# dkogan/libdogleg

Hardware: NVIDIA B200
Metric: dogleg_iterations_per_sec (higher is better)
Workload: dtype f64

## Files before the change

### libdogleg_b200/csrc/dlb_device.h

```cpp
#pragma once
#include <cuda_runtime.h>
#include <cstdint>
#include "dlb_taskplan.h"
#include "dlb_common.cuh"

struct __align__(16) DlbClsInfo { int k, m0, nm, r0; };
struct __align__(16) DlbLeaf { long long off; int c0, nc, r, rp, fcls0, ncls; };
struct __align__(16) DlbSmallTask { int k, m0, nm, r0; long long goff, Goff; };

struct DlbSparseDev
{
  int n, m, ncls, ntasks;
  const int* cls_ptr;
  const int* cls_rows;
  const int* cls_loc;
  const int* cls_front;
  const int* task_cls;
  const int* task_m0;
  const int* task_m1;
  const long long* task_goff;
  const long long* task_Goff;
  const int* mem_col;
  const unsigned int* mem_pos;
  const int* ginv_ptr;
// ... 28 lines not shown
  const int* w;
  const long long* src_ptr;
  const long long* gs_base;
  const int* gs_ld;
};

struct DlbFrontDev
{
  int n, nsuper;
  const int* sn_first;
  const int* rows_ptr;
  const int* rows;
  const int* rel;
  const int* sn_parent;
  const int* child_ptr;
  const int* child_list;
  const long long* front_off;
  const int* fcls_ptr;
  const int* fcls_list;
  const int* cls_task_ptr;
  const int* level_sn;
  const int* perm;
  const DlbLeaf* leaf;
  const unsigned int* leaf_pos; const unsigned int* leaf_kl; const unsigned int* leaf_loc;
  int leaf_ps, leaf_lw;
  int leaf_max_nc;
  long long ytot;
  const long long* heavy_tmp_off;
  double* heavy_tmp;
  DlbGather fg;
  DlbGather sg;
  const char* sg_flag;
};

struct DlbBigFront { long long off; int r, nc, col0, sn; long long inv_off; };

#define DLB_TRIAL_PART 8
#define DLB_TRIAL_PROF_MAX 62
enum { DLB_TRIAL_CAUCHY = 0, DLB_TRIAL_GN = 1, DLB_TRIAL_INTERP = 2 };
struct DlbPublished { DlbScalars sc; unsigned long long seq; };
struct DlbTrial
{
  int nlev; const int* level_ptr; const long long* level_gt; const long long* level_sg; const long long* level_tmp;
  int max_rows, max_cols, any_solve_gather;
  int small_tail;
  const double* Jtx; const double* p_from; const double* Gpart; double* cauchy; double* gn;
  double norm2_Jtx, norm2_cauchy, norm2_gn; int have_cauchy, have_gn;
  double* step; double* p_to; double* h_p_to;
  double* fronts; double* ywork; double* zperm;
  double* part; unsigned int* bar; long long* minor; long long* minor_next;
  DlbScalars* sc; DlbPublished* pub; unsigned long long seq;
  double delta, lambda;
  const int* eg_ptr; const unsigned int* eg_dst; const int* eg_sptr; const int* eg_src;
  unsigned long long* prof;
};
size_t dlb_trial_smem_bytes(int max_rows);
int  dlb_trial_threads(int max_rows);
int  dlb_trial_max_grid(int max_rows, int sm_count);
int  dlb_launch_trial(const DlbSparseDev& S, const DlbFrontDev& F, const DlbTrial& T, int grid, cudaStream_t st);

void dlb_launch_sparse_grad(const DlbSparseDev& S, const double* Jx, const double* x, double* gpart,
                            double* n2part, double* Jtx, double* part, unsigned int* counter,
                            DlbScalars* sc, int sm_count, cudaStream_t st);
int  dlb_sparse_n2part_size(const DlbSparseDev& S, int sm_count);
struct DlbPublished;
int  dlb_launch_sparse_eval_pass(const DlbSparseDev& S, const double* Jx, const double* x, double* Gpart, double* gpart,
                                 double* n2part, int sm_count, cudaStream_t st);
void dlb_launch_sparse_eval_reduce(const DlbSparseDev& S, const double* gpart, const double* n2part, int n2count, double* Jtx,
                                   double* part, unsigned int* counter, DlbScalars* sc, DlbPublished* pub, unsigned long long seq,
                                   int n2_behind_Jtx, int sm_count, cudaStream_t st);
void dlb_launch_sparse_jv(const DlbSparseDev& S, const double* Jx, const double* v, double* part,
                          unsigned int* counter, double* dst, int sm_count, cudaStream_t st);
void dlb_launch_sparse_jv_quad(const DlbSparseDev& S, const double* Jx, const double* Gpart, const double* v, double* part,
                               unsigned int* counter, double* dst, int sm_count, cudaStream_t st);
void dlb_launch_sparse_assemble(const DlbSparseDev& S, const double* Jx, double* Gpart, int all_small,
                                int sm_count, cudaStream_t st);

void dlb_launch_leaf_fronts(const DlbFrontDev& F, const DlbSparseDev& S, int q0, int q1, const double* Jx,
                            double* fronts, double lambda, long long* minor, int max_rows, int eliminate,
                            int sm_count, cudaStream_t st);
void dlb_launch_leaf_fronts_mma(const DlbFrontDev& F, const DlbSparseDev& S, int q0, int q1, const double* Jx,
                                double* fronts, double lambda, long long* minor, int max_rows, int max_pairs, int eliminate,
                                int sm_count, cudaStream_t st);
void dlb_launch_leaf_solve_fwd(const DlbFrontDev& F, int q0, int q1, const double* fronts, const double* rhs,
                               double* ywork, double* zperm, int nrhs, int sm_count, cudaStream_t st);
void dlb_launch_leaf_solve_bwd(const DlbFrontDev& F, int q0, int q1, const double* fronts, double* zperm,
                               int nrhs, int sm_count, cudaStream_t st);

void dlb_launch_front_level(const DlbFrontDev& F, const DlbSparseDev& S, int l0, int l1,
                            double* fronts, const double* Gpart, double lambda,
                            long long* minor, int max_rows, int skip_elimination, cudaStream_t st);
void dlb_bigfront_factor_batch(const DlbBigFront* d_descs, int nfronts, int max_r, int max_nc, double* fronts, double* inv,
                               int* cnt, long long* minor, cudaStream_t st, double* n_launch);
void dlb_launch_extend_gather(const DlbGather& G, long long t0, long long t1, double* pool, int accumulate, cudaStream_t st);
void dlb_launch_zero_bigfronts(const DlbBigFront* d_descs, int nfronts, int max_r, double* fronts, cudaStream_t st);
void dlb_launch_solve_fwd_level(const DlbFrontDev& F, int l0, int l1, const double* fronts,
                                const double* rhs , double* ywork,
                                double* zperm, int nrhs, int max_rows, int max_cols, cudaStream_t st);
void dlb_launch_solve_bwd_level(const DlbFrontDev& F, int l0, int l1, const double* fronts,
                                double* zperm, int nrhs, int max_rows, int max_cols, cudaStream_t st);
void dlb_launch_fronts_to_dense(const DlbFrontDev& F, const double* fronts, double* out, cudaStream_t st);

void dlb_launch_bigsolve_fwd(const DlbFrontDev& F, const DlbBigFront* d_descs, int nfronts, int max_r, int max_nc,
                             const double* fronts, const double* inv, const double* rhs, double* ywork, double* zperm, int nrhs,
                             cudaStream_t st);
long long dlb_bigsolve_partial_size(int r, int nc);
// ... 28 lines not shown
```

### libdogleg_b200/csrc/dlb_engine.cu

```cuda
#include "dlb_common.cuh"
#include "dlb_device.h"
#include "dlb_symbolic.h"
#include "dlb_gatherplan.h"
#include "dlb_taskplan.h"
#include "dogleg_gpu.h"
#include <vector>
#include <string>
#include <cstring>
#include <cstdlib>
#include <climits>
#include <algorithm>
#include <type_traits>
#include <mutex>
#include <chrono>
#include <thread>

static_assert(sizeof(DlbScalars) == sizeof(dlb_scalars_t), "scalar block mirrors must agree");
#define DLB_SMALL_FRONT_MAX 158

static thread_local std::string g_last_error;
static int g_device = 0;
extern "C" const char* dogleg_gpu_last_error(void) { return g_last_error.c_str(); }
extern "C" const char* dogleg_gpu_version(void)    { return "libdogleg-b200 0.1 (sm_100a)"; }
extern "C" void dlb_set_error(const char* msg)     { g_last_error = msg ? msg : ""; }
// ... 85 lines not shown
{
  double *h_p = 0, *h_x = 0, *h_Jtx = 0, *h_cauchy = 0, *h_gn = 0, *h_step = 0, *h_J = 0;
  int    *h_Jp = 0, *h_Ji = 0;
  double *d_p = 0, *d_x = 0, *d_Jtx = 0, *d_cauchy = 0, *d_gn = 0, *d_step = 0, *d_J = 0;
  double norm2_x = 0;
  double* d_G = 0; bool have_G = false;
  double norm2_Jtx = 0, norm2_cauchy = 0, norm2_gn = 0; bool have_cauchy = false, have_gn = false;
};

struct dlb_engine
{
  int type = 0, N = 0, M = 0, packed = 0, upper = 0, device = 0, sm_count = DLB_SM_COUNT_FALLBACK;
  unsigned int nnz = 0;
  size_t Jcount = 0;
  cudaStream_t st = 0;
  cudaStream_t st_copy = 0; cudaEvent_t ev_copy = 0, ev_idle = 0;
  Slot slot[2];
  DlbScalars* d_sc = 0;
  dlb_scalars_t* h_sc = 0;
  DlbPublished* h_pub = 0; DlbPublished* d_pub = 0; unsigned long long seq = 0;
  double* d_part = 0; unsigned int* d_counter = 0;
  long long* d_minor = 0; long long* h_minor = 0;
  DlbSymbolic* sym = 0;
  DlbSparseDev S{}; DlbFrontDev F{};
  std::vector<void*> dev_allocs;
  std::vector<int> level_ptr;
  std::vector<long long> level_gt_ptr;
  std::vector<long long> level_tmp_size;
  std::vector<long long> level_sg_ptr;
  bool any_solve_gather = false;
  std::vector<int> level_mid;
  std::vector<std::vector<DlbBigFront>> level_big;
  std::vector<int> level_big_ptr, level_big_max_r, level_big_max_nc;
  const DlbBigFront* d_big_descs = 0;
  int* d_big_cnt = 0;
  double* d_biginv = 0;
  const long long* d_big_part_off = 0; double* d_big_partial = 0;
  int max_small_rows = 0;
  int max_front_rows = 0, max_front_cols = 0;
  std::vector<int> level_small_rows, level_rows, level_cols;
  int nleaf = 0, leaf_max_rows = 0;
  bool leaf_mma = false;
  int leaf_max_pairs = 0;
  double *d_gpart = 0, *d_n2part = 0, *d_jvpart = 0, *d_fronts = 0, *d_ywork = 0, *d_zperm = 0;
  bool G_shared = false;
  bool G_global = false;
  long long Goff_total = 0;
  bool fused_eval = false, fused_trial = false;
  int trial_grid = 0;
  const int* d_level_ptr = 0; const long long *d_level_gt = 0, *d_level_sg = 0, *d_level_tmp = 0;
  double* d_trial_part = 0; unsigned int* d_bar = 0;
  unsigned int trial_parity = 0; bool minor_dirty = true;
  const int *d_eg_ptr = 0, *d_eg_sptr = 0, *d_eg_src = 0; const unsigned int* d_eg_dst = 0;
  unsigned long long* d_prof = 0;
  double *d_rhs = 0; int rhs_cap = 0;
  bool sharded = false; int M_total = 0, col_begin = 0;
  bool gather = false;
  long long slice_off = 0;
  std::vector<long long> rank_cb, rank_m, rank_off, rank_nnz;
  double* d_fronts_asm = 0;
  double n_allreduce = 0, allreduce_bytes = 0;
  bool pattern_set = false;
  bool pattern_verified = false;
  bool host_inputs = true;
  std::vector<int> pat_sample;
  unsigned long long pat_hash = 0;
  std::vector<int> pat_full_p, pat_full_i;
  std::vector<int> perm_used; int postorder_used = 0;
  double *d_work = 0, *d_xAx = 0;
  int factor_slot = -1; double factor_lambda = 0;
  int asm_slot = 0;
  bool jv_quad = true;
  bool lazy_p = false;
  double n_launch = 0, n_h2d = 0, n_d2h = 0, n_factor = 0;
  bool timing = false; double phase_ms[8] = {0};
  cudaEvent_t ev0 = 0, ev1 = 0;
};

template<class T> static int dev_upload(dlb_engine* e, const std::vector<T>& v, const T** out)
{
  T* d = 0;
  const size_t bytes = std::max<size_t>(v.size(), 1) * sizeof(T);
  CU(cudaMalloc(&d, bytes));
  e->dev_allocs.push_back(d);
  if(!v.empty()) CU(cudaMemcpyAsync(d, v.data(), v.size() * sizeof(T), cudaMemcpyHostToDevice, e->st));
  *out = d;
  return 0;
}
template<class T> static int dev_alloc(dlb_engine* e, size_t count, T** out)
{
  T* d = 0;
  CU(cudaMalloc(&d, std::max<size_t>(count, 1) * sizeof(T)));
  e->dev_allocs.push_back(d);
  *out = d;
  return 0;
}

static int upload_big_descs(dlb_engine* e)
{
  std::vector<DlbBigFront> all;
  const size_t nlev = e->level_big.size();
  e->level_big_ptr.assign(nlev + 1, 0); e->level_big_max_r.assign(nlev, 0); e->level_big_max_nc.assign(nlev, 0);
  for(size_t l = 0; l < nlev; l++)
  {
    for(const DlbBigFront& b : e->level_big[l])
    {
// ... 721 lines not shown
  e->fused_trial = false;
  {
    const char* ft = getenv("DOGLEG_GPU_FUSED_TRIAL");
    bool can = e->fused_eval && !e->gather && e->nleaf == 0 && Y.nlevels > 0 && Y.nlevels <= 256 &&
               Y.max_front_rows <= DLB_SMALL_FRONT_MAX && !(ft && atoi(ft) == 0);
    for(size_t l = 0; can && l < e->level_big.size(); l++) if(!e->level_big[l].empty()) can = false;
    if(can)
    {
      const int limit = dlb_trial_max_grid(Y.max_front_rows, e->sm_count);
      int want = e->sm_count;
      for(int l = 0; l < Y.nlevels; l++) want = std::max(want, Y.level_ptr[l+1] - Y.level_ptr[l]);
      want = std::max(want, (S.nbig + S.nasm_small + dlb_trial_threads(Y.max_front_rows) / 32 - 1) / (dlb_trial_threads(Y.max_front_rows) / 32));
      e->trial_grid = std::min(limit, std::min(want, 4 * e->sm_count));
      if(e->trial_grid >= 1)
      {
        std::vector<long long> lgt(e->level_gt_ptr), lsg(e->level_sg_ptr), ltmp(e->level_tmp_size);
        lgt.resize(2 * (size_t)Y.nlevels + 1, 0); lsg.resize(2 * (size_t)Y.nlevels + 1, 0); ltmp.resize((size_t)Y.nlevels, 0);
        int r2 = 0;
        r2 |= dev_upload(e, Y.level_ptr, &e->d_level_ptr);
        r2 |= dev_upload(e, lgt, &e->d_level_gt); r2 |= dev_upload(e, lsg, &e->d_level_sg); r2 |= dev_upload(e, ltmp, &e->d_level_tmp);
        {
          std::vector<int> eg_ptr(Y.nsuper + 1, 0), eg_sptr{0}, eg_src;
          std::vector<unsigned int> eg_dst;
          struct Ent { unsigned int dst; int src; };
          std::vector<Ent> ents;
          bool fits = Goff < (1ll << 31);
          for(int sn = 0; sn < Y.nsuper && fits; sn++)
          {
            ents.clear();
            for(int ci = Y.fcls_ptr[sn]; ci < Y.fcls_ptr[sn+1]; ci++)
            {
              const int c = Y.fcls_list[ci];
              const int k = Y.cls_ptr[c+1] - Y.cls_ptr[c];
              const int* loc = Y.cls_loc.data() + Y.cls_ptr[c];
              for(int a = 0, q = 0; a < k; a++)
                for(int b = 0; b <= a; b++, q++)
                {
                  const int la = loc[a], lb = loc[b];
                  const unsigned int row = (unsigned int)std::max(la, lb), col = (unsigned int)std::min(la, lb);
                  for(int t = cls_task_ptr[c]; t < cls_task_ptr[c+1]; t++) ents.push_back({row | (col << 16), (int)(task_Goff[t] + q)});
                }
            }
            std::stable_sort(ents.begin(), ents.end(), [](const Ent& x, const Ent& y) { return x.dst < y.dst; });
            for(size_t i = 0; i < ents.size(); i++)
            {
              if(i == 0 || ents[i].dst != ents[i-1].dst) { if(i) eg_sptr.push_back((int)eg_src.size()); eg_dst.push_back(ents[i].dst); }
              eg_src.push_back(ents[i].src);
            }
            if(!ents.empty()) eg_sptr.push_back((int)eg_src.size());
            eg_ptr[sn+1] = (int)eg_dst.size();
            if(eg_src.size() > (size_t)1 << 30) fits = false;
          }
          if(!fits) { g_last_error = "element lists too large"; r2 = 1; }
          r2 |= dev_upload(e, eg_ptr, &e->d_eg_ptr); r2 |= dev_upload(e, eg_dst, &e->d_eg_dst);
          r2 |= dev_upload(e, eg_sptr, &e->d_eg_sptr); r2 |= dev_upload(e, eg_src, &e->d_eg_src);
        }
        r2 |= dev_alloc(e, (size_t)e->trial_grid * DLB_TRIAL_PART, &e->d_trial_part);
        r2 |= dev_alloc(e, (size_t)4, &e->d_bar);
        { const char* pe = getenv("DOGLEG_GPU_TRIAL_PROF"); e->d_prof = 0; if(pe && atoi(pe) != 0) r2 |= dev_alloc(e, (size_t)DLB_TRIAL_PROF_MAX + 1, &e->d_prof); }
        if(r2) { g_last_error = "out of device memory for the trial kernel's workspace"; return -1; }
        CU(cudaMemsetAsync(e->d_bar, 0, 4 * sizeof(unsigned int), e->st));
        e->fused_trial = true;
      }
    }
  }
  CU(cudaStreamSynchronize(e->st));
  e->pattern_set = true;
  e->pattern_verified = true;
  if(verbose)
  {
    const auto t_end = std::chrono::steady_clock::now();
    size_t fr = 0, tot = 0; cudaMemGetInfo(&fr, &tot);
    fprintf(stderr, "libdogleg-b200: pattern N=%d M=%d: %d classes, %d supernodes, %d levels, nnz(L)=%lld, fronts %.2f GB, "
            "max front %d; symbolic %.2f s, index build + upload %.2f s; device memory in use %.1f GB; fused evaluation %d, trial kernel %d (grid %d)\n",
            e->N, Mtot, Y.ncls, Y.nsuper, Y.nlevels, (long long)Y.nnzL(), 8e-9 * (double)Y.front_off[Y.nsuper], Y.max_front_rows,
            std::chrono::duration<double>(t_sym - t_begin).count(), std::chrono::duration<double>(t_end - t_sym).count(),
            1e-9 * (double)(tot - fr), (int)e->fused_eval, (int)e->fused_trial, e->trial_grid);
  }
  return 0;
}

extern "C" int dlb_engine_upload_p(dlb_engine_t* e, int s)
{
  cudaSetDevice(e->device);
  Slot& L = e->slot[s & 1];
  CU(cudaMemcpyAsync(L.d_p, L.h_p, sizeof(double) * e->N, cudaMemcpyHostToDevice, e->st));
  e->n_h2d += sizeof(double) * e->N;
  return 0;
}

static thread_local struct { dlb_engine* e; int slot; size_t wJ, wx; } g_fill = {0, 0, 0, 0};
#define DLB_FILL_MIN_BYTES (1u << 20)
extern "C" void dlb_engine_begin_host_fill(dlb_engine_t* e, int s)
{
  g_fill.e = 0;
  if(!e->host_inputs || e->type == DOGLEG_DENSE_PRODUCTS) return;
  cudaSetDevice(e->device);
  if(cudaEventRecord(e->ev_idle, e->st) != cudaSuccess || cudaStreamWaitEvent(e->st_copy, e->ev_idle, 0) != cudaSuccess) { cudaGetLastError(); return; }
  g_fill.e = e; g_fill.slot = s & 1; g_fill.wJ = 0; g_fill.wx = 0;
}
static void fill_copy_upto(dlb_engine* e, Slot& L, size_t nJ, size_t nx, bool all)
{
  nJ = std::min(nJ, e->Jcount); nx = std::min(nx, (size_t)e->M);
  if(nx > g_fill.wx && (all || (nx - g_fill.wx) * sizeof(double) >= DLB_FILL_MIN_BYTES))
  {
    cudaMemcpyAsync(L.d_x + (e->gather ? e->col_begin : 0) + g_fill.wx, L.h_x + g_fill.wx, sizeof(double) * (nx - g_fill.wx),
                    cudaMemcpyHostToDevice, e->st_copy);
    g_fill.wx = nx;
// ... 605 lines not shown
{
  cudaSetDevice(e->device);
  Slot& A = e->slot[from & 1]; Slot& B = e->slot[to & 1];
  if(ensure_G(e, from)) return -1;
  {
    PhaseTimer tm(e, 6);
    dlb_launch_step(step_type, delta, A.d_p, A.d_Jtx, A.d_cauchy, A.d_gn, e->N, B.d_step, B.d_p,
                    e->d_part, e->d_counter, e->d_sc, e->sm_count, e->st);
    e->n_launch += step_type == DLB_STEP_INTERPOLATED ? 2 : 1;
    if(launch_norm2_Jv(e, A, B.d_step, &e->d_sc->norm2_Jstep)) return -1;
  }
  if(!e->lazy_p)
  {
    PhaseTimer tm(e, 7);
    CU(cudaMemcpyAsync(B.h_p, B.d_p, sizeof(double) * e->N, cudaMemcpyDeviceToHost, e->st));
    e->n_d2h += sizeof(double) * e->N;
  }
  return sync_scalars(e);
}

extern "C" int dlb_engine_has_trial(const dlb_engine_t* e) { return e->fused_trial ? 1 : 0; }
extern "C" int dlb_engine_has_fused_eval(const dlb_engine_t* e) { return e->fused_eval ? 1 : 0; }
extern "C" int dlb_engine_trial(dlb_engine_t* e, int from, int to, double delta, double lambda)
{
  cudaSetDevice(e->device);
  if(!e->fused_trial) { g_last_error = "dlb_engine_trial: this engine has no fused trial kernel (dlb_engine_has_trial)"; return -1; }
  Slot& A = e->slot[from & 1]; Slot& B = e->slot[to & 1];
  if(!A.have_G) { g_last_error = "dlb_engine_trial: the starting point has not been evaluated"; return -1; }
  if(A.have_gn && (e->factor_slot != (from & 1))) A.have_gn = false;
  if(!A.have_gn) e->factor_slot = -1;
  if(e->minor_dirty)
  {
    static const long long big2[2] = {LLONG_MAX, LLONG_MAX};
    CU(cudaMemcpyAsync(e->d_minor, big2, sizeof(big2), cudaMemcpyHostToDevice, e->st));
    e->minor_dirty = false;
  }
  DlbTrial T;
  memset(&T, 0, sizeof(T));
  T.nlev = (int)e->level_ptr.size() - 1; T.level_ptr = e->d_level_ptr; T.level_gt = e->d_level_gt;
  T.level_sg = e->d_level_sg; T.level_tmp = e->d_level_tmp;
  T.max_rows = e->max_front_rows; T.max_cols = e->max_front_cols; T.any_solve_gather = e->any_solve_gather ? 1 : 0;
  T.small_tail = 2 * (size_t)e->N * sizeof(double) <= dlb_trial_smem_bytes(e->max_front_rows) ? 1 : 0;
  T.Jtx = A.d_Jtx; T.p_from = A.d_p; T.Gpart = A.d_G; T.cauchy = A.d_cauchy; T.gn = A.d_gn;
  T.norm2_Jtx = A.norm2_Jtx; T.norm2_cauchy = A.norm2_cauchy; T.norm2_gn = A.norm2_gn;
  T.have_cauchy = A.have_cauchy ? 1 : 0; T.have_gn = A.have_gn ? 1 : 0;
  T.step = B.d_step; T.p_to = B.d_p; T.h_p_to = e->lazy_p ? NULL : B.h_p;
  T.fronts = e->d_fronts; T.ywork = e->d_ywork; T.zperm = e->d_zperm;
  T.part = e->d_trial_part; T.bar = e->d_bar;
  T.minor = e->d_minor + (e->trial_parity & 1); T.minor_next = e->d_minor + ((e->trial_parity + 1) & 1);
  e->trial_parity++;
  T.sc = e->d_sc; T.pub = e->d_pub; T.seq = ++e->seq;
  T.delta = delta; T.lambda = lambda; T.prof = e->d_prof;
  T.eg_ptr = e->d_eg_ptr; T.eg_dst = e->d_eg_dst; T.eg_sptr = e->d_eg_sptr; T.eg_src = e->d_eg_src;
  {
    PhaseTimer tm(e, 4);
    if(dlb_launch_trial(e->S, e->F, T, e->trial_grid, e->st))
    { g_last_error = std::string("cooperative launch of the trial kernel failed: ") + cudaGetErrorString(cudaGetLastError()); return -1; }
    e->n_launch += 1;
  }
  if(wait_published(e)) return -1;
  if(e->d_prof)
  {
    unsigned long long h[DLB_TRIAL_PROF_MAX + 1];
    CU(cudaStreamSynchronize(e->st));
    CU(cudaMemcpy(h, e->d_prof, sizeof(h), cudaMemcpyDeviceToHost));
    const int n = (int)std::min<unsigned long long>(h[DLB_TRIAL_PROF_MAX], DLB_TRIAL_PROF_MAX);
    fprintf(stderr, "libdogleg-b200: trial kernel phases (us):");
    for(int i = 1; i < n; i++) fprintf(stderr, " %.1f", 1e-3 * (double)(h[i] - h[i-1]));
    fprintf(stderr, "  total %.1f\n", n > 0 ? 1e-3 * (double)(h[n-1] - h[0]) : 0.0);
    dlb_trial_dbg_dump();
  }
  if(!e->lazy_p) e->n_d2h += sizeof(double) * e->N;
  const dlb_scalars_t* sc = e->h_sc;
  if(!A.have_cauchy) { A.have_cauchy = true; A.norm2_cauchy = sc->norm2_cauchy; }
  if(sc->minor >= 0) { if(e->factor_slot == (from & 1)) e->factor_slot = -1; e->n_factor += 1; return 0; }
  if(sc->trial_flags != 0.0)
  {
    A.have_gn = true; A.norm2_gn = sc->norm2_gn;
    e->factor_slot = from & 1; e->factor_lambda = lambda; e->asm_slot = from & 1;
    e->n_factor += 1;
  }
  return 0;
}

extern "C" void dlb_engine_set_lazy_p(dlb_engine_t* e, int on) { e->lazy_p = on != 0; }
extern "C" int dlb_engine_download_p(dlb_engine_t* e, int s)
{
  cudaSetDevice(e->device);
  Slot& L = e->slot[s & 1];
  CU(cudaMemcpyAsync(L.h_p, L.d_p, sizeof(double) * e->N, cudaMemcpyDeviceToHost, e->st));
  CU(cudaStreamSynchronize(e->st));
  e->n_d2h += sizeof(double) * e->N;
  return 0;
}

extern "C" int dlb_engine_download(dlb_engine_t* e, int s)
{
  cudaSetDevice(e->device);
  Slot& L = e->slot[s & 1];
  const size_t nb = sizeof(double) * e->N;
  CU(cudaMemcpyAsync(L.h_p, L.d_p, nb, cudaMemcpyDeviceToHost, e->st));
  CU(cudaMemcpyAsync(L.h_Jtx, L.d_Jtx, nb, cudaMemcpyDeviceToHost, e->st));
  CU(cudaMemcpyAsync(L.h_cauchy, L.d_cauchy, nb, cudaMemcpyDeviceToHost, e->st));
  CU(cudaMemcpyAsync(L.h_gn, L.d_gn, nb, cudaMemcpyDeviceToHost, e->st));
  CU(cudaMemcpyAsync(L.h_step, L.d_step, nb, cudaMemcpyDeviceToHost, e->st));
  CU(cudaStreamSynchronize(e->st));
// ... 63 lines not shown
```

### libdogleg_b200/csrc/dlb_trial.cu

```cuda
#ifdef DLB_TRIAL_DEBUG
#define DLB_ELIM_DBG 1
#endif
#include "dlb_common.cuh"
#include "dlb_device.h"
#include "dlb_devfn.cuh"
#include <climits>

__device__ __forceinline__ void grid_barrier(unsigned int* bar)
{
  __syncthreads();
  if(threadIdx.x == 0)
  {
    const unsigned int nb = blockIdx.x == 0 ? 0x80000000u - (gridDim.x - 1) : 1u;
    __threadfence();
    const unsigned int old = atomicAdd(bar, nb);
    while((((old ^ *(volatile unsigned int*)bar) & 0x80000000u) == 0)) { }
    __threadfence();
  }
  __syncthreads();
}

template<int NT>
__device__ __forceinline__ double fold_sum(const double* part, int k, double* sh)
{
  double a = 0.0;
  for(unsigned int b = threadIdx.x; b < gridDim.x; b += NT) a += ((const volatile double*)part)[(size_t)b * DLB_TRIAL_PART + k];
  a = block_sum(a, sh);
  if(threadIdx.x == 0) sh[32] = a;
  __syncthreads();
  a = sh[32];
  __syncthreads();
  return a;
}
template<int NT>
__device__ __forceinline__ double fold_max(const double* part, int k, double* sh)
{
  double a = 0.0;
  for(unsigned int b = threadIdx.x; b < gridDim.x; b += NT) a = fmax(a, ((const volatile double*)part)[(size_t)b * DLB_TRIAL_PART + k]);
  a = block_max(a, sh);
  if(threadIdx.x == 0) sh[32] = a;
  __syncthreads();
  a = sh[32];
  __syncthreads();
  return a;
}
template<int NT>
__device__ __forceinline__ void put_partial(double* part, int k, double v, double* sh, bool is_max = false)
{
  v = is_max ? block_max(v, sh) : block_sum(v, sh);
  if(threadIdx.x == 0) part[(size_t)blockIdx.x * DLB_TRIAL_PART + k] = v;
}

__device__ __forceinline__ void prof_mark(const DlbTrial& T, int& np)
{
  if(T.prof && blockIdx.x == 0 && threadIdx.x == 0 && np < DLB_TRIAL_PROF_MAX)
  {
    unsigned long long t;
    asm volatile("mov.u64 %0, %%globaltimer;" : "=l"(t));
    T.prof[np++] = t;
  }
}

template<int NT>
__device__ __noinline__ void trial_front(const DlbFrontDev* Fp, const DlbTrial* Tp, int s,
                                         double* A, double* dinv, double* sh_red, int* npp)
{
  const DlbFrontDev& F = *Fp; const DlbTrial& T = *Tp; int& np = *npp;
  extern __shared__ double sm[];
  A = sm + (A - sm); dinv = sm + (dinv - sm);
  const int tid = threadIdx.x, lane = tid & 31, w = tid >> 5;
  const int c0 = F.sn_first[s], nc = F.sn_first[s+1] - c0;
  const int rp = F.rows_ptr[s], r = F.rows_ptr[s+1] - rp;
  const int ld = (r + 1) | 1;
  double* Ag = T.fronts + F.front_off[s];
  for(int idx = tid; idx < ld * r; idx += NT) A[idx] = 0.0;
  __syncthreads();
  for(int d0 = T.eg_ptr[s] + tid; d0 < T.eg_ptr[s+1]; d0 += 2 * NT)
  {
    int q0[2], q1[2], idx[2][8]; double g[2][8], acc[2]; unsigned int dd[2];
#pragma unroll
    for(int u = 0; u < 2; u++)
    {
      const bool on = d0 + u * NT < T.eg_ptr[s+1];
      const int d = on ? d0 + u * NT : d0;
      const int a = T.eg_sptr[d], b = T.eg_sptr[d + 1];
      dd[u] = T.eg_dst[d];
      q0[u] = a; q1[u] = on ? b : a;
      acc[u] = 0.0;
    }
    const int nmax = max(q1[0] - q0[0], q1[1] - q0[1]);
    for(int qb = 0; qb < nmax; qb += 8)
    {
#pragma unroll
      for(int u = 0; u < 2; u++)
#pragma unroll
        for(int e = 0; e < 8; e++)
        {
          const int v = T.eg_src[q0[u] + qb + e < q1[u] ? q0[u] + qb + e : q0[u]];
          idx[u][e] = q0[u] + qb + e < q1[u] ? v : -1;
        }
#pragma unroll
      for(int u = 0; u < 2; u++)
#pragma unroll
        for(int e = 0; e < 8; e++) { const double* p = idx[u][e] >= 0 ? T.Gpart + idx[u][e] : g_dlb_zero; g[u][e] = *p; }
#pragma unroll
      for(int u = 0; u < 2; u++)
#pragma unroll
        for(int e = 0; e < 8; e++) acc[u] += g[u][e];
    }
#pragma unroll
    for(int u = 0; u < 2; u++) if(q1[u] > q0[u]) A[(dd[u] & 0xffffu) + (dd[u] >> 16) * ld] = acc[u];
  }
  __syncthreads();
  prof_mark(T, np);
  const long long toff = F.heavy_tmp_off[s];
  const bool gathered = F.sg_flag[s] != 0;
  double* yg = T.ywork + rp;
  if(toff >= 0)
  {
    const double* T0 = F.heavy_tmp + toff;
    for(int idx0 = tid; idx0 < r * r; idx0 += 8 * NT)
    {
      double t[8];
#pragma unroll
      for(int u = 0; u < 8; u++) t[u] = T0[idx0 + u * NT < r * r ? idx0 + u * NT : idx0];
#pragma unroll
      for(int u = 0; u < 8; u++)
      {
        const int idx = idx0 + u * NT;
        const int j = idx / r, i = idx - j * r;
        if(idx < r * r && i >= j) A[i + j * ld] += t[u];
      }
    }
  }
  else
    for(int ch = F.child_ptr[s]; ch < F.child_ptr[s+1]; ch++)
    {
      const int c   = F.child_list[ch];
      const int ncc = F.sn_first[c+1] - F.sn_first[c];
      const int rc  = F.rows_ptr[c+1] - F.rows_ptr[c];
      const int nb  = rc - ncc;
      const double* U = T.fronts + F.front_off[c];
      const int* rel = F.rel + F.rows_ptr[c] + ncc;
      for(int idx = tid; idx < nb * nb; idx += NT)
      {
        const int j = idx / nb, i = idx - j * nb;
        if(i >= j) A[rel[i] + rel[j] * ld] += U[(ncc + i) + (size_t)(ncc + j) * rc];
      }
      __syncthreads();
    }
  for(int i = tid; i < r; i += NT) A[r + i * ld] = (i < nc ? T.Jtx[F.perm[c0 + i]] : 0.0) + (gathered ? yg[i] : 0.0);
  for(int j = tid; j < nc; j += NT) A[j + j * ld] += T.lambda;
  __syncthreads();
  if(!gathered)
    for(int ch = F.child_ptr[s]; ch < F.child_ptr[s+1]; ch++)
    {
      const int c   = F.child_list[ch];
      const int ncc = F.sn_first[c+1] - F.sn_first[c];
      const int rc  = F.rows_ptr[c+1] - F.rows_ptr[c];
      const double* yc = T.ywork + F.rows_ptr[c];
      const int* rel = F.rel + F.rows_ptr[c];
      for(int i = ncc + tid; i < rc; i += NT) A[r + rel[i] * ld] += yc[i];
      __syncthreads();
    }
  prof_mark(T, np);
  const int fail = front_eliminate<NT>(A, r, nc, ld, r + 1, tid, dinv);
  if(fail >= 0)
  {
    if(tid == 0) atomicMin(T.minor, (long long)(c0 + fail));
    return;
  }
  prof_mark(T, np);
  for(int j = tid >> 5; j < r; j += NT / 32)
    for(int i = lane; i < r; i += 32) Ag[i + (size_t)j * r] = A[i + j * ld];
  for(int i = tid; i < r; i += NT) yg[i] = A[r + i * ld];
  if(F.sn_parent[s] >= 0)
  {
    for(int i = tid; i < nc; i += NT) T.zperm[c0 + i] = A[r + i * ld];
    prof_mark(T, np);
    return;
  }
  prof_mark(T, np);
  for(int b0 = ((nc - 1) / 32) * 32; b0 >= 0; b0 -= 32)
  {
    const int bw = nc - b0 < 32 ? nc - b0 : 32;
    for(int cc = w; cc < bw; cc += NT / 32)
    {
      double acc = 0.0;
      for(int i = b0 + bw + lane; i < r; i += 32) acc = fma(A[i + (b0 + cc) * ld], A[r + i * ld], acc);
      acc = warp_sum_all(acc);
      if(lane == 0) sh_red[cc] = acc;
    }
    __syncthreads();
    if(w == 0)
    {
      double v = lane < bw ? A[r + (b0 + lane) * ld] - sh_red[lane] : 0.0;
      const double di = lane < bw ? dinv[b0 + lane] : 0.0;
      for(int j = bw - 1; j >= 0; j--)
      {
        const double xj = __shfl_sync(0xffffffffu, v * di, j);
        if(lane == j) v = xj;
        else if(lane < j) v = fma(-A[(b0 + j) + (b0 + lane) * ld], xj, v);
      }
      if(lane < bw) A[r + (b0 + lane) * ld] = v;
    }
    __syncthreads();
  }
  for(int i = tid; i < nc; i += NT) T.zperm[c0 + i] = A[r + i * ld];
}

template<int NT>
__device__ __noinline__ void trial_front_bwd(const DlbFrontDev* Fp, const DlbTrial* Tp, int s, double* P, double* sh_red)
{
  const DlbFrontDev& F = *Fp; const DlbTrial& T = *Tp;
  const int tid = threadIdx.x, lane = tid & 31, w = tid >> 5;
  const int c0 = F.sn_first[s], nc = F.sn_first[s+1] - c0;
  const int rp = F.rows_ptr[s], r = F.rows_ptr[s+1] - rp;
  const int ld = r | 1;
  double* xs = P + (size_t)ld * nc;
  double* dinv = xs + r;
  const double* Ag = T.fronts + F.front_off[s];
  const int* rows = F.rows + rp;
  for(int idx = tid; idx < r * nc; idx += NT) { const int j = idx / r, i = idx - j * r; P[i + j * ld] = Ag[idx]; }
  for(int i = tid; i < r; i += NT) xs[i] = T.zperm[rows[i]];
  for(int j = tid; j < nc; j += NT) dinv[j] = 1.0 / Ag[j + (size_t)j * r];
  __syncthreads();
  for(int b0 = ((nc - 1) / 32) * 32; b0 >= 0; b0 -= 32)
  {
    const int bw = nc - b0 < 32 ? nc - b0 : 32;
    for(int cc = w; cc < bw; cc += NT / 32)
    {
      double acc = 0.0;
      for(int i = b0 + bw + lane; i < r; i += 32) acc = fma(P[i + (b0 + cc) * ld], xs[i], acc);
      acc = warp_sum_all(acc);
      if(lane == 0) sh_red[cc] = acc;
    }
    __syncthreads();
    if(w == 0)
    {
      double v = lane < bw ? xs[b0 + lane] - sh_red[lane] : 0.0;
      const double di = lane < bw ? dinv[b0 + lane] : 0.0;
      for(int j = bw - 1; j >= 0; j--)
      {
        const double xj = __shfl_sync(0xffffffffu, v * di, j);
        if(lane == j) v = xj;
        else if(lane < j) v = fma(-P[(b0 + j) + (b0 + lane) * ld], xj, v);
      }
      if(lane < bw) xs[b0 + lane] = v;
    }
    __syncthreads();
  }
  for(int i = tid; i < nc; i += NT) T.zperm[c0 + i] = xs[i];
  __syncthreads();
}

__device__ __noinline__ void ph_gather(const DlbGather* G, long long t0, long long t1, double* pool, int accumulate, int lane,
                                       long long skip)
{
  const long long nw = (long long)gridDim.x * (blockDim.x >> 5);
  const long long wid = (long long)(threadIdx.x >> 5) * gridDim.x + blockIdx.x;
  gather_targets(*G, t0, t1, pool, accumulate, (wid + nw - skip % nw) % nw, nw, lane);
}
__device__ __noinline__ double ph_quadform(const DlbSparseDev* S, const double* Gpart, const double* v, int wid, int nw, int lane)
{
  return quadform_partial(*S, S->big_tasks, S->nbig, S->asm_small_tasks, S->nasm_small, Gpart, v, wid, nw, lane);
}
struct TrialShared { DlbSparseDev S; DlbFrontDev F; DlbTrial T; };

template<int NT>
__global__ void __launch_bounds__(NT, NT == 256 ? 2 : 1)
k_trial(DlbSparseDev S, DlbFrontDev F, DlbTrial T)
{
  __shared__ TrialShared shp;
  if(threadIdx.x == 0) shp.S = S;
  if(threadIdx.x == 32) shp.F = F;
  if(threadIdx.x == 64 % NT) shp.T = T;
  __syncthreads();
  int np = 1;
  if(T.prof && blockIdx.x == 0 && threadIdx.x == 0) { unsigned long long t; asm volatile("mov.u64 %0, %%globaltimer;" : "=l"(t)); T.prof[0] = t; }
#define PROF_MARK() prof_mark(T, np)
  extern __shared__ double sm[];
  __shared__ double sh_red[33];
  const int tid = threadIdx.x, lane = tid & 31;
  const int wid = blockIdx.x * (NT / 32) + (tid >> 5), nw = gridDim.x * (NT / 32);
  const int gtid = blockIdx.x * NT + tid, gnt = gridDim.x * NT;
  const int N = S.n;
  double* part = T.part;
  const double d2 = T.delta * T.delta;

  if(blockIdx.x == 0 && tid == 0) *T.minor_next = LLONG_MAX;

  const bool factorize = !T.have_gn;
  if(!T.have_cauchy) put_partial<NT>(part, 0, ph_quadform(&shp.S, T.Gpart, T.Jtx, wid, nw, lane), sh_red);
  if(factorize)
    for(int q = T.level_ptr[0] + blockIdx.x; q < T.level_ptr[1]; q += gridDim.x)
    {
      trial_front<NT>(&shp.F, &shp.T, F.level_sn[q], sm, sm + (size_t)(T.max_rows + 2) * T.max_rows, sh_red, &np);
      __syncthreads();
    }
  if(!T.have_cauchy || factorize) grid_barrier(T.bar);
  PROF_MARK();

  double n2c, kc = 0.0;
  if(!T.have_cauchy)
  {
    const double jg2 = fold_sum<NT>(part, 0, sh_red);
    const double g2 = T.norm2_Jtx;
    kc = -g2 / jg2;
    n2c = kc * kc * g2;
    for(int i = gtid; i < N; i += gnt) T.cauchy[i] = kc * T.Jtx[i];
    if(blockIdx.x == 0 && tid == 0) { T.sc->norm2_JJtx = jg2; T.sc->k_cauchy = kc; T.sc->norm2_cauchy = n2c; }
  }
  else n2c = T.norm2_cauchy;

  const bool want_gn = !(n2c >= d2);
  double n2gn = T.have_gn ? T.norm2_gn : 0.0;
  long long minor_seen = LLONG_MAX;
  if(want_gn && factorize)
  {
    minor_seen = *(volatile long long*)T.minor;
    for(int l = 1; l < T.nlev && minor_seen == LLONG_MAX; l++)
    {
      const long long g0 = T.level_gt[2*l], g1 = T.level_gt[2*l+1], g2 = T.level_gt[2*l+2];
      const long long s0 = T.level_sg[2*l], s1 = T.level_sg[2*l+1], s2 = T.level_sg[2*l+2];
      if(g2 > g0 || s2 > s0)
      {
        for(long long i = gtid; i < T.level_tmp[l]; i += gnt) F.heavy_tmp[i] = 0.0;
        for(int q = T.level_ptr[l] + blockIdx.x; q < T.level_ptr[l+1]; q += gridDim.x)
        {
          const int sq = F.level_sn[q];
          if(F.sg_flag[sq]) for(int i = F.rows_ptr[sq] + tid; i < F.rows_ptr[sq+1]; i += NT) T.ywork[i] = 0.0;
        }
        ph_gather(&shp.F.fg, g0, g1, T.fronts, 0, lane, 0);
        ph_gather(&shp.F.sg, s0, s1, T.ywork, 0, lane, g1 - g0);
        grid_barrier(T.bar);
        PROF_MARK();
        ph_gather(&shp.F.fg, g1, g2, T.fronts, 1, lane, 0);
        ph_gather(&shp.F.sg, s1, s2, T.ywork, 1, lane, g2 - g1);
        grid_barrier(T.bar);
        PROF_MARK();
      }
      for(int q = T.level_ptr[l] + blockIdx.x; q < T.level_ptr[l+1]; q += gridDim.x)
      {
        trial_front<NT>(&shp.F, &shp.T, F.level_sn[q], sm, sm + (size_t)(T.max_rows + 2) * T.max_rows, sh_red, &np);
        __syncthreads();
      }
      grid_barrier(T.bar);
      PROF_MARK();
      minor_seen = *(volatile long long*)T.minor;
    }
    if(minor_seen == LLONG_MAX)
      for(int l = T.nlev - 2; l >= 0; l--)
      {
        for(int q = T.level_ptr[l] + blockIdx.x; q < T.level_ptr[l+1]; q += gridDim.x)
        {
          const int s = F.level_sn[q];
          if(F.sn_parent[s] < 0) continue;
          trial_front_bwd<NT>(&shp.F, &shp.T, s, sm, sh_red);
        }
        grid_barrier(T.bar);
        PROF_MARK();
      }
  }
  if(minor_seen != LLONG_MAX)
  {
    if(blockIdx.x == 0 && tid == 0)
    {
      T.sc->minor = minor_seen; T.sc->trial_flags = 0.0;
      DlbPublished* pub = T.pub;
      pub->sc = *T.sc;
      __threadfence_system();
      *(volatile unsigned long long*)&pub->seq = T.seq;
    }
    return;
  }
  const bool fresh_gn = want_gn && factorize;

  if(T.small_tail)
  {
    double* sgn = sm; double* sstep = sm + N;
    if(want_gn)
    {
      if(fresh_gn)
      {
        double n2 = 0.0;
        for(int k = tid; k < N; k += NT) { const double v = -T.zperm[k]; sgn[F.perm[k]] = v; n2 = fma(v, v, n2); }
        n2 = block_sum(n2, sh_red);
        if(tid == 0) sh_red[32] = n2;
        __syncthreads();
        n2gn = sh_red[32];
        __syncthreads();
        if(blockIdx.x == 0) { for(int i = tid; i < N; i += NT) T.gn[i] = sgn[i]; if(tid == 0) T.sc->norm2_gn = n2gn; }
      }
      else { for(int i = tid; i < N; i += NT) sgn[i] = T.gn[i]; __syncthreads(); }
    }
    const int type = !want_gn ? DLB_TRIAL_CAUCHY : (n2gn <= d2 ? DLB_TRIAL_GN : DLB_TRIAL_INTERP);
    double kI = 0.0, disc_raw = 0.0;
// ... 194 lines not shown
```

Before: 2339.

## Precompute upper-level element sums during first phase and add blocked root factorization

The per-element Gpart sums for fronts above the leaf level are now computed by the whole grid in a new phase that runs before the leaf fronts, and stored in an esum buffer. Upper-level fronts then scatter these precomputed sums instead of gathering and summing in their own critical path. Root fronts get a dedicated blocked Cholesky routine that uses DMMA updates with 8-wide panels and a warp-level triangular solve, replacing the generic eliminate plus the 32-wide back-substitution. Level-1 zeroing is also moved into the early phase. The cost is an extra buffer, extra work in the first phase, and more complex root code with a risk of numerical or indexing differences.

```diff
diff --git a/libdogleg_b200/csrc/dlb_device.h b/libdogleg_b200/csrc/dlb_device.h
--- a/libdogleg_b200/csrc/dlb_device.h
+++ b/libdogleg_b200/csrc/dlb_device.h
@@ -104,6 +104,7 @@
   DlbScalars* sc; DlbPublished* pub; unsigned long long seq;
   double delta, lambda;
   const int* eg_ptr; const unsigned int* eg_dst; const int* eg_sptr; const int* eg_src;
+  const int* eg_up; int n_eg_up; double* esum;
   unsigned long long* prof;
 };
 size_t dlb_trial_smem_bytes(int max_rows);
diff --git a/libdogleg_b200/csrc/dlb_engine.cu b/libdogleg_b200/csrc/dlb_engine.cu
--- a/libdogleg_b200/csrc/dlb_engine.cu
+++ b/libdogleg_b200/csrc/dlb_engine.cu
@@ -161,6 +161,7 @@
   double* d_trial_part = 0; unsigned int* d_bar = 0;
   unsigned int trial_parity = 0; bool minor_dirty = true;
   const int *d_eg_ptr = 0, *d_eg_sptr = 0, *d_eg_src = 0; const unsigned int* d_eg_dst = 0;
+  const int* d_eg_up = 0; int n_eg_up = 0; double* d_esum = 0;
   unsigned long long* d_prof = 0;
   double *d_rhs = 0; int rhs_cap = 0;
   bool sharded = false; int M_total = 0, col_begin = 0;
@@ -988,8 +989,13 @@
             if(eg_src.size() > (size_t)1 << 30) fits = false;
           }
           if(!fits) { g_last_error = "element lists too large"; r2 = 1; }
+          std::vector<int> eg_up;
+          for(int q = Y.nlevels > 1 ? Y.level_ptr[1] : 0; Y.nlevels > 1 && q < Y.level_ptr[Y.nlevels]; q++)
+            for(int d = eg_ptr[Y.level_sn[q]]; d < eg_ptr[Y.level_sn[q] + 1]; d++) eg_up.push_back(d);
+          e->n_eg_up = (int)eg_up.size();
           r2 |= dev_upload(e, eg_ptr, &e->d_eg_ptr); r2 |= dev_upload(e, eg_dst, &e->d_eg_dst);
           r2 |= dev_upload(e, eg_sptr, &e->d_eg_sptr); r2 |= dev_upload(e, eg_src, &e->d_eg_src);
+          r2 |= dev_upload(e, eg_up, &e->d_eg_up); r2 |= dev_alloc(e, eg_dst.size(), &e->d_esum);
         }
         r2 |= dev_alloc(e, (size_t)e->trial_grid * DLB_TRIAL_PART, &e->d_trial_part);
         r2 |= dev_alloc(e, (size_t)4, &e->d_bar);
@@ -1701,6 +1707,7 @@
   T.sc = e->d_sc; T.pub = e->d_pub; T.seq = ++e->seq;
   T.delta = delta; T.lambda = lambda; T.prof = e->d_prof;
   T.eg_ptr = e->d_eg_ptr; T.eg_dst = e->d_eg_dst; T.eg_sptr = e->d_eg_sptr; T.eg_src = e->d_eg_src;
+  T.eg_up = e->d_eg_up; T.n_eg_up = e->n_eg_up; T.esum = e->d_esum;
   {
     PhaseTimer tm(e, 4);
     if(dlb_launch_trial(e->S, e->F, T, e->trial_grid, e->st))
diff --git a/libdogleg_b200/csrc/dlb_trial.cu b/libdogleg_b200/csrc/dlb_trial.cu
--- a/libdogleg_b200/csrc/dlb_trial.cu
+++ b/libdogleg_b200/csrc/dlb_trial.cu
@@ -61,20 +61,222 @@
   }
 }
 
+__device__ __forceinline__ void root_invert_diag(double* A, int ld, int b0, int bw, const double* dinv, int lane)
+{
+  if(lane >= bw) return;
+  double x[8];
+#pragma unroll
+  for(int i = 0; i < 8; i++)
+  {
+    double t = i == lane ? 1.0 : 0.0;
+#pragma unroll
+    for(int m = 0; m < i; m++) t = fma(-A[(b0 + (i < bw ? i : 0)) + (size_t)(b0 + (i < bw ? m : 0)) * ld], x[m], t);
+    x[i] = t * dinv[b0 + (i < bw ? i : 0)];
+  }
+#pragma unroll
+  for(int i = 1; i < 8; i++)
+    if(i > lane && i < bw) A[(b0 + lane) + (size_t)(b0 + i) * ld] = x[i];
+}
+
 template<int NT>
-__device__ __noinline__ void trial_front(const DlbFrontDev* Fp, const DlbTrial* Tp, int s,
+__device__ __forceinline__ int root_eliminate(double* A, int n, int ld, double* dinv, volatile int* sh_fail)
+{
+  constexpr int NW = NT / 32;
+  const int tid = threadIdx.x, lane = tid & 31, w = tid >> 5;
+  const int g = lane >> 2, tt = lane & 3;
+  const int nrows = n + 1;
+  __syncthreads();
+  for(int b0 = 0; b0 < n; b0 += 8)
+  {
+    const int bw = n - b0 < 8 ? n - b0 : 8;
+    if(b0 > 0)
+    {
+      const int ntr = (nrows - b0 + 7) >> 3;
+      const int rb = b0 + g < n ? b0 + g : n - 1;
+      const int cj = b0 + 2 * tt;
+      for(int ti0 = w; ti0 < ntr; ti0 += 4 * NW)
+      {
+        int ri[4], ric[4]; double c0[4], c1[4], d0[4], d1[4];
+#pragma unroll
+        for(int u = 0; u < 4; u++)
+        {
+          ri[u] = b0 + 8 * (ti0 + NW * u) + g;
+          ric[u] = ri[u] < nrows ? ri[u] : nrows - 1;
+          c0[u] = 0.0; c1[u] = 0.0; d0[u] = 0.0; d1[u] = 0.0;
+        }
+        for(int k = 0; k < b0; k += 8)
+        {
+          const size_t ko = (size_t)(k + tt) * ld, kp = ko + 4 * (size_t)ld;
+          const double vb = A[rb + ko], wb = A[rb + kp];
+          double va[4], wa[4];
+#pragma unroll
+          for(int u = 0; u < 4; u++) { va[u] = A[ric[u] + ko]; wa[u] = A[ric[u] + kp]; }
+#pragma unroll
+          for(int u = 0; u < 4; u++) { devfn_dmma(c0[u], c1[u], va[u], vb); devfn_dmma(d0[u], d1[u], wa[u], wb); }
+        }
+#pragma unroll
+        for(int u = 0; u < 4; u++)
+          if(ti0 + NW * u < ntr && ri[u] < nrows)
+          {
+            if(cj < b0 + bw && (ri[u] >= cj || ri[u] >= n))         A[ri[u] + (size_t)cj * ld]       -= c0[u] + d0[u];
+            if(cj + 1 < b0 + bw && (ri[u] >= cj + 1 || ri[u] >= n)) A[ri[u] + (size_t)(cj + 1) * ld] -= c1[u] + d1[u];
+          }
+      }
+      __syncthreads();
+    }
+    if(w == 0)
+    {
+      double L[36], rs[8];
+#pragma unroll
+      for(int i = 0; i < 8; i++)
+#pragma unroll
+        for(int j = 0; j <= i; j++)
+        {
+          const double val = A[(b0 + (i < bw ? i : 0)) + (size_t)(b0 + (i < bw ? j : 0)) * ld];
+          L[i * (i + 1) / 2 + j] = i < bw ? val : (i == j ? 1.0 : 0.0);
+        }
+      int fail = -1;
+#pragma unroll
+      for(int j = 0; j < 8; j++)
+      {
+        const double d = L[j * (j + 1) / 2 + j];
+        if((!(d > 0.0) || isinf(d)) && fail < 0) fail = b0 + j;
+        rs[j] = rsqrt(d);
+        L[j * (j + 1) / 2 + j] = d * rs[j];
+#pragma unroll
+        for(int i = j + 1; i < 8; i++) L[i * (i + 1) / 2 + j] *= rs[j];
+#pragma unroll
+        for(int i = j + 1; i < 8; i++)
+#pragma unroll
+          for(int c = j + 1; c <= i; c++)
+            L[i * (i + 1) / 2 + c] = fma(-L[i * (i + 1) / 2 + j], L[c * (c + 1) / 2 + j], L[i * (i + 1) / 2 + c]);
+      }
+      if(lane < bw)
+      {
+#pragma unroll
+        for(int i = 0; i < 8; i++)
+          if(i == lane)
+          {
+#pragma unroll
+            for(int j = 0; j <= i; j++) A[(b0 + i) + (size_t)(b0 + j) * ld] = L[i * (i + 1) / 2 + j];
+            dinv[b0 + i] = rs[i];
+          }
+      }
+      if(lane == 0) *sh_fail = fail;
+    }
+    __syncthreads();
+    const int fail = *sh_fail;
+    if(fail >= 0) return fail;
+    if(b0 + bw + tid < nrows)
+    {
+      double L[36], rs[8];
+#pragma unroll
+      for(int i = 0; i < 8; i++)
+      {
+#pragma unroll
+        for(int j = 0; j < i; j++) L[i * (i + 1) / 2 + j] = A[(b0 + (i < bw ? i : 0)) + (size_t)(b0 + (i < bw ? j : 0)) * ld];
+        rs[i] = dinv[b0 + (i < bw ? i : 0)];
+      }
+      for(int i = b0 + bw + tid; i < nrows; i += NT)
+      {
+        double x[8], v[8];
+#pragma unroll
+        for(int c = 0; c < 8; c++) v[c] = A[i + (size_t)(b0 + (c < bw ? c : 0)) * ld];
+#pragma unroll
+        for(int c = 0; c < 8; c++)
+        {
+          double t = c < bw ? v[c] : 0.0;
+#pragma unroll
+          for(int cp = 0; cp < c; cp++) t = fma(-x[cp], L[c * (c + 1) / 2 + cp], t);
+          x[c] = t * rs[c];
+          if(c < bw) A[i + (size_t)(b0 + c) * ld] = x[c];
+        }
+      }
+    }
+    if(w == NW - 1) root_invert_diag(A, ld, b0, bw, dinv, lane);
+    __syncthreads();
+  }
+  return -1;
+}
+
+template<int NT>
+__device__ __noinline__ int trial_root(double* A, int n, int ld, double* dinv, double* Ag, double* yg, double* z,
+                                       double* sh_red, const DlbTrial* Tp, int* npp)
+{
+  constexpr int NW = NT / 32;
+  extern __shared__ double sm[];
+  A = sm + (A - sm); dinv = sm + (dinv - sm);
+  const int tid = threadIdx.x, lane = tid & 31, w = tid >> 5;
+  const int nb = (n + 7) >> 3;
+  const int fail = root_eliminate<NT>(A, n, ld, dinv, (volatile int*)sh_red);
+  prof_mark(*Tp, *npp);
+  if(fail >= 0) return fail;
+  double* y = A + n;
+  if(w == 0)
+  {
+    for(int i = lane; i < n; i += 32) yg[i] = y[(size_t)i * ld];
+    __syncwarp();
+    for(int k = nb - 1; k >= 0; k--)
+    {
+      const int b0 = 8 * k, bw = min(8, n - b0);
+      const int c = lane < bw ? lane : 0;
+      double x = dinv[b0 + c] * y[(size_t)(b0 + c) * ld];
+#pragma unroll
+      for(int m = 1; m < 8; m++)
+      {
+        const bool on = c + m < bw;
+        const int i = on ? c + m : c;
+        const double xi = A[(b0 + c) + (size_t)(b0 + i) * ld];
+        x = fma(on ? xi : 0.0, y[(size_t)(b0 + i) * ld], x);
+      }
+      __syncwarp();
+      if(lane < bw) y[(size_t)(b0 + lane) * ld] = x;
+      double xs[8];
+#pragma unroll
+      for(int i = 0; i < 8; i++) { const double v = __shfl_sync(0xffffffffu, x, i); xs[i] = i < bw ? v : 0.0; }
+      for(int cc = lane; cc < b0; cc += 32)
+      {
+        double v = y[(size_t)cc * ld];
+#pragma unroll
+        for(int i = 0; i < 8; i++) v = fma(-A[(b0 + (i < bw ? i : 0)) + (size_t)cc * ld], xs[i], v);
+        y[(size_t)cc * ld] = v;
+      }
+      __syncwarp();
+    }
+    for(int i = lane; i < n; i += 32) z[i] = y[(size_t)i * ld];
+  }
+  else
+  {
+    for(int j = w - 1; j < n; j += NW - 1)
+      for(int i = lane; i < n; i += 32) Ag[i + (size_t)j * n] = i >= j ? A[i + (size_t)j * ld] : 0.0;
+  }
+  return -1;
+}
+
+template<int NT>
+__device__ __noinline__ void trial_front(const DlbFrontDev* Fp, const DlbTrial* Tp, int s, bool summed,
                                          double* A, double* dinv, double* sh_red, int* npp)
 {
   const DlbFrontDev& F = *Fp; const DlbTrial& T = *Tp; int& np = *npp;
   extern __shared__ double sm[];
   A = sm + (A - sm); dinv = sm + (dinv - sm);
-  const int tid = threadIdx.x, lane = tid & 31, w = tid >> 5;
+  const int tid = threadIdx.x, lane = tid & 31;
   const int c0 = F.sn_first[s], nc = F.sn_first[s+1] - c0;
   const int rp = F.rows_ptr[s], r = F.rows_ptr[s+1] - rp;
   const int ld = (r + 1) | 1;
   double* Ag = T.fronts + F.front_off[s];
   for(int idx = tid; idx < ld * r; idx += NT) A[idx] = 0.0;
   __syncthreads();
+  if(summed)
+    for(int d0 = T.eg_ptr[s] + tid; d0 < T.eg_ptr[s+1]; d0 += 8 * NT)
+    {
+      unsigned int dd[8]; double v[8];
+#pragma unroll
+      for(int u = 0; u < 8; u++) { const int d = d0 + u * NT < T.eg_ptr[s+1] ? d0 + u * NT : d0; dd[u] = T.eg_dst[d]; v[u] = T.esum[d]; }
+#pragma unroll
+      for(int u = 0; u < 8; u++) if(d0 + u * NT < T.eg_ptr[s+1]) A[(dd[u] & 0xffffu) + (dd[u] >> 16) * ld] = v[u];
+    }
+  else
   for(int d0 = T.eg_ptr[s] + tid; d0 < T.eg_ptr[s+1]; d0 += 2 * NT)
   {
     int q0[2], q1[2], idx[2][8]; double g[2][8], acc[2]; unsigned int dd[2];
@@ -164,6 +366,13 @@
       __syncthreads();
     }
   prof_mark(T, np);
+  if(F.sn_parent[s] < 0)
+  {
+    const int fail = trial_root<NT>(A, r, ld, dinv, Ag, yg, T.zperm + c0, sh_red, Tp, npp);
+    if(fail >= 0 && tid == 0) atomicMin(T.minor, (long long)(c0 + fail));
+    prof_mark(T, np);
+    return;
+  }
   const int fail = front_eliminate<NT>(A, r, nc, ld, r + 1, tid, dinv);
   if(fail >= 0)
   {
@@ -174,39 +383,8 @@
   for(int j = tid >> 5; j < r; j += NT / 32)
     for(int i = lane; i < r; i += 32) Ag[i + (size_t)j * r] = A[i + j * ld];
   for(int i = tid; i < r; i += NT) yg[i] = A[r + i * ld];
-  if(F.sn_parent[s] >= 0)
-  {
-    for(int i = tid; i < nc; i += NT) T.zperm[c0 + i] = A[r + i * ld];
-    prof_mark(T, np);
-    return;
-  }
+  for(int i = tid; i < nc; i += NT) T.zperm[c0 + i] = A[r + i * ld];
   prof_mark(T, np);
-  for(int b0 = ((nc - 1) / 32) * 32; b0 >= 0; b0 -= 32)
-  {
-    const int bw = nc - b0 < 32 ? nc - b0 : 32;
-    for(int cc = w; cc < bw; cc += NT / 32)
-    {
-      double acc = 0.0;
-      for(int i = b0 + bw + lane; i < r; i += 32) acc = fma(A[i + (b0 + cc) * ld], A[r + i * ld], acc);
-      acc = warp_sum_all(acc);
-      if(lane == 0) sh_red[cc] = acc;
-    }
-    __syncthreads();
-    if(w == 0)
-    {
-      double v = lane < bw ? A[r + (b0 + lane) * ld] - sh_red[lane] : 0.0;
-      const double di = lane < bw ? dinv[b0 + lane] : 0.0;
-      for(int j = bw - 1; j >= 0; j--)
-      {
-        const double xj = __shfl_sync(0xffffffffu, v * di, j);
-        if(lane == j) v = xj;
-        else if(lane < j) v = fma(-A[(b0 + j) + (b0 + lane) * ld], xj, v);
-      }
-      if(lane < bw) A[r + (b0 + lane) * ld] = v;
-    }
-    __syncthreads();
-  }
-  for(int i = tid; i < nc; i += NT) T.zperm[c0 + i] = A[r + i * ld];
 }
 
 template<int NT>
@@ -265,6 +443,41 @@
 {
   return quadform_partial(*S, S->big_tasks, S->nbig, S->asm_small_tasks, S->nasm_small, Gpart, v, wid, nw, lane);
 }
+__device__ __noinline__ void ph_zero_level(const DlbTrial* Tp, const DlbFrontDev* Fp, int l)
+{
+  const DlbTrial& T = *Tp; const DlbFrontDev& F = *Fp;
+  const long long gtid = (long long)blockIdx.x * blockDim.x + threadIdx.x, gnt = (long long)gridDim.x * blockDim.x;
+  for(long long i = gtid; i < T.level_tmp[l]; i += gnt) F.heavy_tmp[i] = 0.0;
+  for(int q = T.level_ptr[l] + blockIdx.x; q < T.level_ptr[l+1]; q += gridDim.x)
+  {
+    const int sq = F.level_sn[q];
+    if(F.sg_flag[sq]) for(int i = F.rows_ptr[sq] + threadIdx.x; i < F.rows_ptr[sq+1]; i += blockDim.x) T.ywork[i] = 0.0;
+  }
+}
+__device__ __noinline__ void ph_elements(const DlbTrial* Tp, const DlbFrontDev* Fp)
+{
+  const DlbTrial& T = *Tp;
+  ph_zero_level(Tp, Fp, 1);
+  const int nwb = blockDim.x >> 5;
+  const int slot = (threadIdx.x & 31) * nwb + (threadIdx.x >> 5);
+  for(int e = slot * gridDim.x + blockIdx.x; e < T.n_eg_up; e += gridDim.x * blockDim.x)
+  {
+    const int d = T.eg_up[e];
+    const int q0 = T.eg_sptr[d], q1 = T.eg_sptr[d + 1];
+    double acc = 0.0;
+    for(int qb = q0; qb < q1; qb += 8)
+    {
+      int idx[8]; double g[8];
+#pragma unroll
+      for(int u = 0; u < 8; u++) { const int v = T.eg_src[qb + u < q1 ? qb + u : q0]; idx[u] = qb + u < q1 ? v : -1; }
+#pragma unroll
+      for(int u = 0; u < 8; u++) { const double* p = idx[u] >= 0 ? T.Gpart + idx[u] : g_dlb_zero; g[u] = *p; }
+#pragma unroll
+      for(int u = 0; u < 8; u++) acc += g[u];
+    }
+    T.esum[d] = acc;
+  }
+}
 struct TrialShared { DlbSparseDev S; DlbFrontDev F; DlbTrial T; };
 
 template<int NT>
@@ -291,11 +504,12 @@
   if(blockIdx.x == 0 && tid == 0) *T.minor_next = LLONG_MAX;
 
   const bool factorize = !T.have_gn;
+  if(factorize && T.nlev > 1) ph_elements(&shp.T, &shp.F);
   if(!T.have_cauchy) put_partial<NT>(part, 0, ph_quadform(&shp.S, T.Gpart, T.Jtx, wid, nw, lane), sh_red);
   if(factorize)
     for(int q = T.level_ptr[0] + blockIdx.x; q < T.level_ptr[1]; q += gridDim.x)
     {
-      trial_front<NT>(&shp.F, &shp.T, F.level_sn[q], sm, sm + (size_t)(T.max_rows + 2) * T.max_rows, sh_red, &np);
+      trial_front<NT>(&shp.F, &shp.T, F.level_sn[q], false, sm, sm + (size_t)(T.max_rows + 2) * T.max_rows, sh_red, &np);
       __syncthreads();
     }
   if(!T.have_cauchy || factorize) grid_barrier(T.bar);
@@ -325,12 +539,7 @@
       const long long s0 = T.level_sg[2*l], s1 = T.level_sg[2*l+1], s2 = T.level_sg[2*l+2];
       if(g2 > g0 || s2 > s0)
       {
-        for(long long i = gtid; i < T.level_tmp[l]; i += gnt) F.heavy_tmp[i] = 0.0;
-        for(int q = T.level_ptr[l] + blockIdx.x; q < T.level_ptr[l+1]; q += gridDim.x)
-        {
-          const int sq = F.level_sn[q];
-          if(F.sg_flag[sq]) for(int i = F.rows_ptr[sq] + tid; i < F.rows_ptr[sq+1]; i += NT) T.ywork[i] = 0.0;
-        }
+        if(l > 1) ph_zero_level(&shp.T, &shp.F, l);
         ph_gather(&shp.F.fg, g0, g1, T.fronts, 0, lane, 0);
         ph_gather(&shp.F.sg, s0, s1, T.ywork, 0, lane, g1 - g0);
         grid_barrier(T.bar);
@@ -342,7 +551,7 @@
       }
       for(int q = T.level_ptr[l] + blockIdx.x; q < T.level_ptr[l+1]; q += gridDim.x)
       {
-        trial_front<NT>(&shp.F, &shp.T, F.level_sn[q], sm, sm + (size_t)(T.max_rows + 2) * T.max_rows, sh_red, &np);
+        trial_front<NT>(&shp.F, &shp.T, F.level_sn[q], true, sm, sm + (size_t)(T.max_rows + 2) * T.max_rows, sh_red, &np);
         __syncthreads();
       }
       grid_barrier(T.bar);
```

Measured after the change: 2310, median of 6. About the same (-1.2%).
